# omar-a-aman/Franka-Force-Feedback-MPC

Measured on AMD Instinct MI355X. Metric: FDDP solves/sec, Franka 7-DoF horizon-30 batch=4096, at 1/2/4/8 MI355X, higher is better.
Workload: dtype f64

## Files before the change

franka-force-feedback-mpc_amd/csrc/ffddp_kernels.hip:

```cpp
#include <hip/hip_runtime.h>
#include <sched.h>

#include <cmath>
#include <cstdio>
#include <cstdlib>
#include <cstring>
#include <new>
#include <algorithm>
#include <atomic>
#include <chrono>
#include <condition_variable>
#include <functional>
#include <mutex>
#include <string>
#include <thread>
#include <type_traits>
#include <vector>

#include "ffddp_consts.hpp"
#include "ffddp_group.hpp"
#include "ffddp_plant.hpp"
#include "ffddp_primal_g8.hpp"
#include "ffddp_rollout.hpp"

// ... 28 lines not shown
#define BW_WAVES 1
#endif

struct InstState {
  double preg, cost, dg, dq, stop;
  double ffeas;
  int is_feasible, was_feasible, done, ok, iter, recalc, accepted, bw_ok;
  int n_iters, n_trials, n_retries, n_backward, n_calc, n_forward;
  int n_eval1, n_eval2;
  int n_neg, n_neg_acc;
};

struct Dev {
  int B, N, nx, rec;
  double* rec_buf;
  double* fs;
  double* xs;
  double* us;
  double* K;
  double* k;
  double* w;
  double* xs_try;
  double* us_try;
  double* trial;
  int* trial_fail;
  InstState* st;
  int* alist;
  int* acnt;
  double* trace;
  int trace_it;
};

#define RESERVE_AGPR40() asm volatile("" ::: "a0", "a1", "a2", "a3", "a4", "a5", "a6", "a7", "a8", "a9", "a10", "a11", "a12", "a13", "a14", "a15", "a16", "a17", "a18", "a19", "a20", "a21", "a22", "a23", "a24", "a25", "a26", "a27", "a28", "a29", "a30", "a31", "a32", "a33", "a34", "a35", "a36", "a37", "a38", "a39")

template <class T> using gptr = __attribute__((address_space(1))) T*;

struct ActiveList {
  const int* list;
  int n;
};
__device__ __forceinline__ ActiveList active_list(const Dev& d, int cur) {
  return ActiveList{d.alist + (long)cur * d.B, d.acnt[cur]};
}

constexpr int N_XCD = 8;
__device__ __forceinline__ long xcd_block(long b, long n) {
  if (b >= n) return b;
  const long q = n / N_XCD, r = n % N_XCD;
  const long x = b % N_XCD, i = b / N_XCD;
  return (x < r ? x * (q + 1) : r * (q + 1) + (x - r) * q) + i;
}

__global__ void k_init(const DevConsts* __restrict__ Cg, Dev d, const double* xs_init, const double* us_init,
                       int is_feasible) {
  const DevConsts& C = *Cg;
  const int N = C.N, nx = C.nx;
  const long nX = (long)d.B * (N + 1) * nx;
  const long nU = (long)d.B * N * NU;
  const long nK = (long)d.B * N * NU * nx;
  const long nT = d.trace ? (long)d.B * d.trace_it * FFDDP_TRACE_W : 0;
  for (long i = blockIdx.x * (long)blockDim.x + threadIdx.x; i < nK || i < nT; i += (long)gridDim.x * blockDim.x) {
    if (i < nT) d.trace[i] = __builtin_nan("");
    if (i >= nK) continue;
    if (i < nX) d.xs[i] = xs_init[i];
    if (i < nU) {
      d.us[i] = us_init[i];
      d.k[i] = 0.0;
    }
    d.K[i] = 0.0;
    if (i < d.B) {
      d.alist[i] = (int)i;
      if (i == 0) {
        d.acnt[0] = d.B;
        d.acnt[1] = 0;
        d.acnt[2] = 0;
        d.acnt[3] = 0;
      }
      InstState s;
      s.preg = C.reg_min;
      s.cost = 0.0;
      s.dg = s.dq = 0.0;
      s.stop = __builtin_nan("");
      s.is_feasible = is_feasible;
      s.was_feasible = 0;
      s.done = 0;
      s.ok = 0;
      s.iter = 0;
      s.recalc = 1;
      s.accepted = -1;
      s.bw_ok = 0;
      s.n_iters = s.n_trials = s.n_retries = s.n_backward = s.n_calc = s.n_forward = 0;
      s.n_eval1 = s.n_eval2 = 0;
      s.n_neg = s.n_neg_acc = 0;
      s.ffeas = 0.0;
      d.st[i] = s;
    }
  }
}

struct NodeGroupShared {
  Primal P;
  union {
    double lk[LK_ALLOC];
    double col[14][NDENSE_MAX];
  };
  double colu[7][FFDDP_MAX_NC];
};
struct NodeShared {
  NodeGroupShared g[NODE_GPB];
};

template <int NC, bool FF>
__device__ __forceinline__ void primal_group(const DevConsts& C, const Dev& d, const double* __restrict__ x0,
                                             const double* __restrict__ node_ref, const double* __restrict__ inst_ref,
                                             const uint8_t* __restrict__ surface, int b, int t, Primal* P,
                                             double* lk, const double* __restrict__ xsrc,
                                             const double* __restrict__ usrc) {
  const int N = C.N;
  constexpr int nx = FF ? 21 : 14;
// ... 47 lines not shown
        }
      }
    }
    c += g8_sum(part);
  }
  if (li == 0) {
    rec[rec_off_cost(nx)] = c;
#pragma unroll
    for (int r = 0; r < 3; ++r) rec[rec_off_lam(nx) + r] = (mode == MODE_TERMINAL_X) ? 0.0 : lam[r];
  }
  const bool feas = d.st[b].is_feasible != 0;
  if (J) {
    if (!terminal) {
      double* f = d.fs + ((long)b * (N + 1) + t + 1) * nx;
      const double* yn = xsrc + (long)(t + 1) * nx;
      const double dt = C.dt;
      const double a = P->a[li];
      const double qn = (mode == MODE_TERMINAL_X) ? q : q + (v * dt + a * dt * dt);
      const double vn = (mode == MODE_TERMINAL_X) ? v : v + a * dt;
      f[li] = feas ? 0.0 : qn - yn[li];
      f[7 + li] = feas ? 0.0 : vn - yn[7 + li];
      if (FF) f[14 + li] = feas ? 0.0 : (C.alpha * y[14 + li] + C.beta * usrc[(long)t * NU + li]) - yn[14 + li];
    }
    if (t == 0) {
      double* f = d.fs + (long)b * (N + 1) * nx;
#pragma unroll
      for (int k = 0; k < (FF ? 3 : 2); ++k) f[7 * k + li] = feas ? 0.0 : x0[(long)b * nx + 7 * k + li] - y[7 * k + li];
    }
  }
  if (!FF && commit) {
    double* xr = d.xs + ((long)b * (N + 1) + t) * nx;
    xr[li] = q;
    xr[7 + li] = v;
    if (!terminal) d.us[((long)b * N + t) * NU + li] = cu;
  }
}

template <int NC>
__device__ __forceinline__ double fquad(const double* a, const double* Dd, const double* Do, const double* b) {
  double acc = 0.0;
#pragma unroll
  for (int r = 0; r < NC; ++r) acc += a[r] * Dd[r] * b[r];
  if (NC == 3)
    acc += Do[0] * (a[1] * b[0] + a[0] * b[1]) + Do[1] * (a[2] * b[0] + a[0] * b[2]) +
           Do[2] * (a[2] * b[1] + a[1] * b[2]);
  return acc;
}

template <int NC, bool FF>
__global__ __launch_bounds__(NODE_BLOCK) __attribute__((amdgpu_waves_per_eu(NODE_WAVES))) void k_node(const DevConsts* __restrict__ Cg, Dev d,
                                                      const double* __restrict__ x0,
                                                      const double* __restrict__ node_ref,
                                                      const double* __restrict__ inst_ref,
                                                      const uint8_t* __restrict__ surface, int force_all, int cur) {
  const DevConsts& C = *Cg;
  const int N = C.N;
  constexpr int nx = FF ? 21 : 14;
  constexpr int nc = NC;
  __shared__ NodeShared S;
  const int grp = threadIdx.x / NODE_GROUP, lane = threadIdx.x % NODE_GROUP;
  const int n_work = force_all ? d.B : d.acnt[cur];
  const long blk = xcd_block(blockIdx.x, ((long)n_work * (N + 1) + NODE_GPB - 1) / NODE_GPB);
  const long gnode = blk * NODE_GPB + grp;
  const int slot = (int)(gnode / (N + 1)), t = (int)(gnode % (N + 1));
  int b = slot;
  bool active = slot < d.B;
  if (active && !force_all) {
    const ActiveList al = active_list(d, cur);
    active = slot < al.n;
    b = active ? al.list[slot] : 0;
    if (active) active = (d.st[b].done == 0) && (d.st[b].recalc != 0);
  }
  const long node = (long)b * (N + 1) + t;
  const bool surf = active ? surface[b] != 0 : false;
  const bool terminal = t == N;
  constexpr bool ff = FF;
  const int mode = !terminal ? MODE_RUNNING : (ff ? MODE_TERMINAL_U : MODE_TERMINAL_X);
  const long perX = (long)(N + 1) * nx, perU = (long)N * NU;
  const int acc = active ? d.st[b].accepted : -1;
  const double* xsrc = acc >= 0 ? d.xs_try + ((long)b * NTRIALS + acc) * perX : d.xs + (long)b * perX;
  const double* usrc = acc >= 0 ? d.us_try + ((long)b * NTRIALS + acc) * perU : d.us + (long)b * perU;
  const double* y = xsrc + (long)t * nx;
  const double* ref = node_ref + ((long)b * (N + 1) + t) * 6;
  NodeGroupShared& G = S.g[grp];
  Primal& P = G.P;
  if (active && lane < G8) primal_group<NC, FF>(C, d, x0, node_ref, inst_ref, surface, b, t, &P, G.lk, xsrc, usrc);
  __syncthreads();
  const bool need_u = mode != MODE_TERMINAL_X;
  if (active && lane < 7 && need_u) {
    double dau[NQ], dlamu[3];
    node_tangent_control<NC>(C, surf, P, lane, dau, dlamu);
    double* rec = d.rec_buf + ((long)b * (N + 1) + t) * d.rec;
    for (int i = 0; i < NQ; ++i) rec[rec_off_A() + (14 + lane) * NQ + i] = dau[i];
    for (int r = 0; r < nc; ++r) G.colu[lane][r] = (surf ? dlamu[r] : 0.0);
  }
  double da[NQ], dlam[3], col[NDENSE_MAX], r1[NQ], dh[3];
  if (active && lane < 14) node_tangent_state_links<NC>(C, mode, surf, G.lk, P, lane, r1, dh, col);
  __syncthreads();
  if (active && lane < 14) {
    for (int r = 0; r < 12; ++r) G.col[lane][r] = col[r];
    node_tangent_state_contact<NC>(mode, surf, P, r1, dh, da, dlam, col);
    for (int r = 12; r < 12 + nc; ++r) G.col[lane][r] = col[r];
  }
  __syncthreads();
  if (active) {
    double* rec = d.rec_buf + ((long)b * (N + 1) + t) * d.rec;
    const int nd = 12 + nc;
    const bool scale = mode != MODE_TERMINAL_X;
    const double sc = scale ? C.dt : 1.0;
    const double* D = P.D;
    const double* g = P.g;
    double wy = 0.0, wy2j = 0.0, wy2u = 0.0;
    if (ff) {
      wy = C.w_y;
      wy2j = C.Wy2[lane < 14 ? lane : 0];
      wy2u = C.Wy2[14 + (lane < 7 ? lane : 0)];
      asm volatile("" : "+s"(wy), "+v"(wy2j), "+v"(wy2u));
    }
    if (lane < 14) {
      const int j = lane;
      if (need_u)
        for (int i = 0; i < NQ; ++i) rec[rec_off_A() + j * NQ + i] = da[i];
      double* Lxx = rec + rec_off_Lxx(nx);
      for (int i = 0; i < 14; ++i) {
        double acc = 0.0;
        for (int r = 0; r < 12; ++r) acc += G.col[i][r] * D[r] * col[r];
        acc += fquad<NC>(&G.col[i][12], D + 12, P.Dfo, col + 12);
        if (i == j) acc += P.Dx[j];
        acc *= sc;
        if (ff && i == j) acc += wy * wy2j;
        Lxx[i * nx + j] = acc;
      }
      double lx = 0.0;
      for (int r = 0; r < nd; ++r) lx += col[r] * g[r];
// ... 1473 lines not shown
  if (steplength > C.th_stepdec) s.preg = fmax(s.preg / C.reg_dec, C.reg_min);
  if (steplength <= C.th_stepinc) {
    s.preg = fmin(s.preg * C.reg_inc, C.reg_max);
    if (s.preg == C.reg_max) {
      s.done = 1;
      s.ok = 0;
    }
  }
  if (d.trace && iter < d.trace_it && !s.done) {
    double* r = d.trace + ((long)b * d.trace_it + iter) * FFDDP_TRACE_W;
    r[0] = (double)iter;
    r[1] = s.cost;
    r[2] = s.stop;
    r[3] = -td1;
    r[4] = s.preg;
    r[5] = s.preg;
    r[6] = steplength;
    r[7] = s.ffeas;
    r[8] = tdV;
    r[9] = tdVexp;
  }
  if (!s.done && s.was_feasible && s.stop < C.th_stop) {
    s.done = 1;
    s.ok = 1;
  }
  d.st[b] = s;
  return acc;
}

__global__ __launch_bounds__(64) void k_accept(const DevConsts* __restrict__ Cg, Dev d, int iter, int n1, int cur,
                                               int wide_max) {
  const DevConsts& C = *Cg;
  const ActiveList al = active_list(d, cur);
  const int n1h = n1;
  n1 = first_width(n1, d, cur, wide_max);
  if ((int)blockIdx.x * 64 >= al.n) return;
  const int slot = (int)blockIdx.x * 64 + (int)threadIdx.x;
  const bool has = slot < al.n;
  const int b = has ? al.list[slot] : 0;
  bool cont = false;
  int acc = -1;
  if (has) {
    acc = accept_instance(C, d, b, iter, n1);
    cont = d.st[b].done == 0;
  }
  if (cont && (acc < 0 || acc >= n1h)) d.acnt[2 + (cur ^ 1)] = 1;
  const unsigned long long m = __ballot(cont);
  int base = 0;
  if (threadIdx.x == 0 && m != 0ull) base = atomicAdd(d.acnt + (cur ^ 1), __popcll(m));
  base = __builtin_amdgcn_readfirstlane(base);
  if (cont) d.alist[(long)(cur ^ 1) * d.B + base + __popcll(m & ((1ull << threadIdx.x) - 1ull))] = b;
}

constexpr int COMMIT_IPB = 4;
__global__ __launch_bounds__(64) void k_commit(const DevConsts* __restrict__ Cg, Dev d) {
  const DevConsts& C = *Cg;
  const int q = threadIdx.x / 16, l = threadIdx.x % 16;
  const int b = (int)blockIdx.x * COMMIT_IPB + q;
  if (b >= d.B) return;
  const int acc = d.st[b].accepted;
  if (acc < 0) return;
  const int N = C.N, nx = C.nx;
  const long perX = (long)(N + 1) * nx, perU = (long)N * NU;
  const double* sx = d.xs_try + ((long)b * NTRIALS + acc) * perX;
  const double* su = d.us_try + ((long)b * NTRIALS + acc) * perU;
  double* dx = d.xs + (long)b * perX;
  double* du = d.us + (long)b * perU;
  constexpr int CH = 16;
  for (long base = l; base < perX + perU; base += 16 * CH) {
    double v[CH];
#pragma unroll
    for (int u = 0; u < CH; ++u) {
      const long i = base + 16 * u;
      v[u] = i < perX ? sx[i] : (i < perX + perU ? su[i - perX] : 0.0);
    }
#pragma unroll
    for (int u = 0; u < CH; ++u) {
      const long i = base + 16 * u;
      if (i < perX)
        dx[i] = v[u];
      else if (i < perX + perU)
        du[i - perX] = v[u];
    }
  }
}

template <int NC, bool FF>
__global__ __launch_bounds__(64) void k_finalize(const DevConsts* __restrict__ Cg, Dev d, int maxiter, const double* __restrict__ x0,
                           const double* __restrict__ node_ref, const double* __restrict__ inst_ref,
                           const uint8_t* __restrict__ surface, double* cost, int32_t* iters, uint8_t* ok,
                           double* fn_pred, int32_t* stats) {
  const DevConsts& C = *Cg;
  const int N = C.N;
  constexpr int nx = FF ? 21 : 14;
  const long gid = blockIdx.x * (long)blockDim.x + threadIdx.x;
  const int b = (int)(gid / 2), knot = (int)(gid % 2);
  if (b >= d.B) return;
  const InstState s = d.st[b];
  if (knot == 0) {
    cost[b] = s.cost;
    iters[b] = s.done ? s.iter : maxiter;
    ok[b] = (s.done && s.ok) ? 1 : 0;
    if (stats) {
      stats[(long)b * FFDDP_NSTATS + 0] = s.n_iters;
      stats[(long)b * FFDDP_NSTATS + 1] = s.n_trials;
      stats[(long)b * FFDDP_NSTATS + 2] = s.n_retries;
      stats[(long)b * FFDDP_NSTATS + 3] = s.n_backward;
      stats[(long)b * FFDDP_NSTATS + 4] = s.n_calc;
      stats[(long)b * FFDDP_NSTATS + 5] = s.n_forward;
      stats[(long)b * FFDDP_NSTATS + 6] = s.n_eval1;
      stats[(long)b * FFDDP_NSTATS + 7] = s.n_eval2;
      stats[(long)b * FFDDP_NSTATS + 8] = s.n_neg;
      stats[(long)b * FFDDP_NSTATS + 9] = s.n_neg_acc;
    }
  }
  if (fn_pred == nullptr) return;
  const int t = knot < N ? knot : N - 1;
  if (!surface[b]) {
    fn_pred[(long)b * 2 + knot] = __builtin_nan("");
    return;
  }
  const double* y = d.xs + ((long)b * (N + 1) + t) * nx;
  const double* u = d.us + ((long)b * N + t) * NU;
  const double* ref = node_ref + ((long)b * (N + 1) + t) * 6;
  const double* xreg = inst_ref + (long)b * 21;
  Primal P;
  double yn[21], c;
  node_calc<NC, FF>(C, false, true, y, u, ref, xreg, xreg + 14, x0 + (long)b * nx, P, yn, c);
  fn_pred[(long)b * 2 + knot] = (NC == 1) ? P.lam[0] : P.lam[2];
}

__global__ __launch_bounds__(64) void k_plant(const ffddp_robot* __restrict__ rb, const ffddp_plant_params* __restrict__ pp,
                                              int B, double* __restrict__ q, double* __restrict__ v,
                                              const double* __restrict__ tau, const double* __restrict__ plane,
                                              int integrate, double* __restrict__ obs, int32_t* __restrict__ fail) {
  const int b = blockIdx.x * blockDim.x + threadIdx.x;
  if (b >= B) return;
  double qb[NQ], vb[NQ], tb[NQ], ob[PO_WORDS];
  for (int i = 0; i < NQ; ++i) {
    qb[i] = q[(long)b * NQ + i];
    vb[i] = v[(long)b * NQ + i];
    tb[i] = tau[(long)b * NQ + i];
  }
  const double* pl = plane + (long)b * 6;
  const bool ok = plant_step(*rb, *pp, qb, vb, tb, pl, pl + 3, integrate, ob);
  for (int i = 0; i < NQ; ++i) {
    q[(long)b * NQ + i] = qb[i];
    v[(long)b * NQ + i] = vb[i];
  }
  for (int e = 0; e < PO_WORDS; ++e) obs[(long)b * PO_WORDS + e] = ob[e];
  if (fail) fail[b] = ok ? 0 : 1;
}

__global__ __launch_bounds__(64) void k_gravity(const ffddp_robot* __restrict__ rb, int B, const double* __restrict__ q,
                          double* __restrict__ tau) {
  const int b = blockIdx.x * blockDim.x + threadIdx.x;
  if (b >= B) return;
  gravity_torque(*rb, q + (long)b * NQ, tau + (long)b * NQ);
}

struct TaskTraj {
  double center[3], radius, omega, z_contact, t_approach, t_pre, t_hold;
  double p_start[3], p_pre[3], p_cs[3];
};

__device__ __forceinline__ double smoothstep01(double s) {
  s = fmin(fmax(s, 0.0), 1.0);
  return s * s * (3.0 - 2.0 * s);
}

__device__ __forceinline__ double dsmoothstep01(double s) {
  s = fmin(fmax(s, 0.0), 1.0);
  return 6.0 * s * (1.0 - s);
}

__device__ bool task_base(const TaskTraj& T, double t, double p[3], double v[3]) {
// ... 222 lines not shown
    uint64_t seen = 0;
    for (;;) {
      {
        std::unique_lock<std::mutex> lk(mu_);
        cv_.wait(lk, [&] { return stop_ || (gen_ != seen && work_ != nullptr); });
        if (stop_) return;
        seen = gen_;
      }
      drain();
    }
  }
  std::vector<std::thread> th_;
  std::mutex mu_;
  std::condition_variable cv_, done_cv_;
  const std::vector<CopyJob>* work_ = nullptr;
  std::atomic<size_t> next_{0};
  size_t left_ = 0;
  uint64_t gen_ = 0;
  bool stop_ = false;
};

struct ffddp_handle {
  int device = 0;
  int max_batch = 0;
  DevConsts hc{};
  DevConsts* dc = nullptr;
  ffddp_robot* drb = nullptr;
  Dev d{};
  double *in_x0 = nullptr, *in_nref = nullptr, *in_iref = nullptr, *in_xs = nullptr, *in_us = nullptr;
  uint8_t* in_surf = nullptr;
  double *out_xs = nullptr, *out_us = nullptr, *out_K = nullptr, *out_cost = nullptr, *out_fn = nullptr;
  int32_t *out_iters = nullptr, *out_stats = nullptr;
  uint8_t* out_ok = nullptr;
  std::string err;
  char* stage = nullptr;
  size_t stage_bytes = 0;
  std::vector<hipEvent_t> hdone;
  CopyPool* pool = nullptr;
  double* trace = nullptr;
  int trace_it = 0;
  std::vector<ffddp_plan*> plans;
  hipEvent_t last_done = nullptr;
  bool last_done_set = false;
  int nstreams = 4;
  std::vector<hipStream_t> streams;
  std::vector<hipEvent_t> sev;
  std::vector<hipEvent_t> stg;
  bool caller_slice = true;
  int stagger = -1;
  int fw_first = 4;
  std::vector<int> fw_sched{2, 2, 2, 2};
  int bw_late_max = -1;
  int bw_w2_max = -1;
  int n_simd = 1024;
  bool fw_fill = true;
  int fw_long = 0;
  int fw_wide_max = -1;
  int ls_row_max = -1;
  bool prof = false;
  int prof_mask = 0;
  std::vector<hipEvent_t> ev_pool;
  size_t ev_used = 0;
  std::vector<int> ev_class;
  double prof_ms[FFDDP_NKERNELS] = {0};
  int64_t prof_n[FFDDP_NKERNELS] = {0};
};

namespace {

bool stream_pool_acquire(int device, int n, std::vector<hipStream_t>& out);
void stream_pool_release(int device, int n);


int fail(ffddp_handle* h, int code, const std::string& msg) {
  if (h) h->err = msg;
  return code;
}

#define HIPCHK(h, expr)                                                                    \
  do {                                                                                     \
    hipError_t e_ = (expr);                                                                \
    if (e_ != hipSuccess)                                                                  \
      return fail(h, FFDDP_E_DEVICE, std::string(#expr) + ": " + hipGetErrorString(e_));  \
  } while (0)

template <class T> int dalloc(ffddp_handle* h, T** p, size_t n) {
  if (hipMalloc((void**)p, n * sizeof(T) + 64) != hipSuccess) {
    *p = nullptr;
    return fail(h, FFDDP_E_OOM, "hipMalloc failed");
  }
  return 0;
}

void free_all(ffddp_handle* h) {
  void* ps[] = {h->dc, h->drb, h->d.alist, h->d.acnt, h->d.rec_buf, h->d.fs, h->d.xs, h->d.us, h->d.K, h->d.k, h->d.w, h->d.xs_try,
                h->d.us_try, h->d.trial, h->d.trial_fail, h->d.st, h->in_x0, h->in_nref, h->in_iref, h->in_xs,
                h->in_us, h->in_surf, h->out_xs, h->out_us, h->out_K, h->out_cost, h->out_fn, h->out_iters,
                h->out_stats, h->out_ok};
  for (void* p : ps)
    if (p) (void)hipFree(p);
  if (h->trace) (void)hipFree(h->trace);
  if (h->stage) (void)hipHostFree(h->stage);
}

struct ProfScope {
  ffddp_handle* h;
// ... 40 lines not shown
  d.acnt += 4 * k;
  if (d.trace) d.trace += (long)b0 * d0.trace_it * FFDDP_TRACE_W;
  return d;
}

template <int NC, bool FF>
int launch_solve_t(ffddp_handle* h, int B, const double* x0, const double* nref, const double* iref,
                 const uint8_t* surf, const double* xs_init, const double* us_init, int maxiter, int is_feasible,
                 double* xs, double* us, double* K, double* cost, int32_t* iters, uint8_t* ok, double* fn_pred,
                 int32_t* stats, hipStream_t s, HostIO* io) {
  const int N = h->hc.N, nx = h->hc.nx;
  int S = h->nstreams;
  if (B < 64 * S) S = 1;
  if (S > 1) {
    if ((int)h->streams.size() < S && !stream_pool_acquire(h->device, S, h->streams))
      return fail(h, FFDDP_E_DEVICE, "hipStreamCreate failed");
    while ((int)h->sev.size() < S + 1) {
      hipEvent_t e;
      HIPCHK(h, hipEventCreateWithFlags(&e, hipEventDisableTiming));
      h->sev.push_back(e);
    }
    while ((int)h->stg.size() < S) {
      hipEvent_t e;
      HIPCHK(h, hipEventCreateWithFlags(&e, hipEventDisableTiming));
      h->stg.push_back(e);
    }
  }
  const int Bs = (B + S - 1) / S;
  const int stagger = S == 1 ? 0 : (h->stagger >= 0 ? h->stagger : (Bs > h->n_simd / S ? 1 : 0));
  struct Slice {
    Dev d;
    hipStream_t s;
    int b0, B;
  };
  Slice sl[8];
  Dev dbase = h->d;
  if (!io) {
    dbase.xs = xs;
    dbase.us = us;
    dbase.K = K;
  }
  for (int k = 0; k < S; ++k) {
    sl[k].b0 = k * Bs;
    sl[k].B = (B - sl[k].b0) < Bs ? (B - sl[k].b0) : Bs;
    sl[k].d = dev_slice(dbase, sl[k].b0, sl[k].B, k);
    sl[k].s = (S > 1 && !(h->caller_slice && k == S - 1)) ? h->streams[k] : s;
  }
  if (S > 1) {
    HIPCHK(h, hipEventRecord(h->sev[0], s));
    for (int k = 0; k < S; ++k)
      if (sl[k].s != s) HIPCHK(h, hipStreamWaitEvent(sl[k].s, h->sev[0], 0));
  }
  const long nxl = nx, N1 = N + 1;
  if (io) {
    io->ns = S;
    for (int k = 0; k < S; ++k) {
      io->b0[k] = sl[k].b0;
      io->bk[k] = sl[k].B;
    }
  }
  auto enqueue_in = [&](int k) -> int {
    for (int i = 0; i < io->n_in; ++i) {
      const size_t o = (size_t)sl[k].b0 * io->in[i].per_inst;
      HIPCHK(h, hipMemcpyAsync((char*)io->in[i].dev + o, (const char*)io->in[i].host + o,
                               (size_t)sl[k].B * io->in[i].per_inst, hipMemcpyHostToDevice, sl[k].s));
    }
    return 0;
  };
  auto enqueue_init = [&](int k) {
    ProfScope p(h, sl[k].s, KC_INIT);
    const long b0 = sl[k].b0;
    hipLaunchKernelGGL(k_init, dim3(1024), dim3(256), 0, sl[k].s, h->dc, sl[k].d, xs_init + b0 * N1 * nxl,
                       us_init + b0 * (long)N * NU, is_feasible);
  };
  auto enqueue_iter = [&](int k, int it) -> int {
    const Dev& d = sl[k].d;
    const hipStream_t ss = sl[k].s;
    const int Bk = sl[k].B;
    const long b0 = sl[k].b0;
    const double* x0k = x0 + b0 * nxl;
    const double* nrefk = nref + b0 * N1 * 6;
    const double* irefk = iref + b0 * 21;
    const uint8_t* surfk = surf + b0;
    const long nodes = (long)Bk * (N + 1);
    if (it == 0 && k > 0 && stagger) HIPCHK(h, hipStreamWaitEvent(ss, h->stg[k - 1], 0));
    if (it == 0 && stagger == 2 && k + 1 < S) HIPCHK(h, hipEventRecord(h->stg[k], ss));
    {
      ProfScope p(h, ss, KC_NODE);
      hipLaunchKernelGGL((k_node<NC, FF>), dim3((int)((nodes + NODE_GPB - 1) / NODE_GPB)), dim3(NODE_BLOCK), 0, ss,
                         h->dc, d, x0k, nrefk, irefk, surfk, 0, it & 1);
    }
    if (it == 0 && stagger == 1 && k + 1 < S) HIPCHK(h, hipEventRecord(h->stg[k], ss));
    {
      ProfScope p(h, ss, KC_BACKWARD);
      const int lmax = h->bw_late_max >= 0 ? h->bw_late_max : h->n_simd / S;
      const bool small = Bk <= h->n_simd / S;
      const int w2auto = small ? h->n_simd / (2 * S) : (FF ? 0 : lmax);
      const int w2max = std::min(lmax, h->bw_w2_max >= 0 ? h->bw_w2_max : w2auto);
      if (lmax < Bk)
        hipLaunchKernelGGL((k_backward_w<FF>), dim3(Bk), dim3(64), 0, ss, h->dc, d, it, it & 1, lmax, w2max);
      if (lmax > w2max && w2max < Bk)
        hipLaunchKernelGGL((k_backward_w<FF, true>), dim3(lmax < Bk ? lmax : Bk), dim3(64), 0, ss, h->dc, d, it, it & 1,
                           lmax, w2max);
      if (w2max > 0) {
        const dim3 g2(w2max < Bk ? w2max : Bk);
        if constexpr (!FF) {
          if (!small) {
            hipLaunchKernelGGL((k_backward_w2<FF, 2>), g2, dim3(128), 0, ss, h->dc, d, it, it & 1, w2max);
          } else {
            hipLaunchKernelGGL((k_backward_w2<FF, 1>), g2, dim3(128), 0, ss, h->dc, d, it, it & 1, w2max);
          }
        } else {
          hipLaunchKernelGGL((k_backward_w2<FF, 1>), g2, dim3(128), 0, ss, h->dc, d, it, it & 1, w2max);
        }
      }
    }
    int n1 = NTRIALS;
    {
      n1 = it < (int)h->fw_sched.size() ? h->fw_sched[it] : h->fw_first;
      if (h->fw_fill) n1 = std::max(n1, std::min(NTRIALS, 8 * h->n_simd / std::max(B, 1)));
      if (h->fw_fill && h->fw_long > 0 && N >= h->fw_long && n1 >= 8) n1 = NTRIALS;
      const int wide = h->fw_wide_max >= 0 ? h->fw_wide_max : h->n_simd / S;
      const long g1 = std::max((long)Bk * n1, (long)std::min(Bk, wide) * NTRIALS);
      const int row_max = (h->ls_row_max >= 0 ? h->ls_row_max : 4 * h->n_simd / S) *
                          (h->ls_row_max < 0 && Bk > h->n_simd / S ? 0 : 1);
      const bool row_only = row_max > 0 && (long)Bk * NTRIALS <= (long)row_max;
      auto fw = [&](int tr0, int ntr, int more) {
        const long groups = more ? (long)Bk * ntr : g1;
        if (!row_only) {
          const dim3 grid((unsigned)((groups * G8 + 63) / 64));
          hipLaunchKernelGGL((k_forward_g8<NC, FF, false>), grid, dim3(64), 0, ss, h->dc, d, x0k, nrefk, irefk,
                             surfk, tr0, ntr, more, it & 1, wide, row_max);
        }
        if (row_max > 0) {
          const long rg = std::min(groups, (long)row_max);
          const dim3 grid((unsigned)((rg * 16 + 63) / 64));
          hipLaunchKernelGGL((k_forward_g8<NC, FF, true>), grid, dim3(64), 0, ss, h->dc, d, x0k, nrefk, irefk,
                             surfk, tr0, ntr, more, it & 1, wide, row_max);
        }
      };
      {
        ProfScope p(h, ss, KC_FORWARD);
        fw(0, n1, 0);
      }
      if (n1 < NTRIALS) {
        ProfScope p(h, ss, KC_FORWARD2);
        fw(n1, NTRIALS - n1, 1);
      }
    }
    {
      ProfScope p(h, ss, KC_ACCEPT);
      hipLaunchKernelGGL(k_accept, dim3((Bk + 63) / 64), dim3(64), 0, ss, h->dc, d, it, n1, it & 1,
                         h->fw_wide_max >= 0 ? h->fw_wide_max : h->n_simd / S);
    }
    return 0;
  };
  const size_t bxs = (size_t)(N + 1) * nx * sizeof(double);
  const size_t bus = (size_t)N * NU * sizeof(double);
  const size_t bks = (size_t)N * NU * nx * sizeof(double);
  auto enqueue_tail = [&](int k) -> int {
    const Dev& d = sl[k].d;
    const hipStream_t ss = sl[k].s;
    const long b0 = sl[k].b0;
    const int Bk = sl[k].B;
    {
      ProfScope p(h, ss, KC_COMMIT);
      hipLaunchKernelGGL(k_commit, dim3((Bk + COMMIT_IPB - 1) / COMMIT_IPB), dim3(64), 0, ss, h->dc, d);
    }
    {
      ProfScope p(h, ss, KC_FINALIZE);
      hipLaunchKernelGGL((k_finalize<NC, FF>), dim3((2 * Bk + 63) / 64), dim3(64), 0, ss, h->dc, d, maxiter,
                         x0 + b0 * nxl, nref + b0 * N1 * 6, iref + b0 * 21, surf + b0, cost + b0, iters + b0, ok + b0,
                         fn_pred ? fn_pred + 2 * b0 : nullptr, stats ? stats + b0 * FFDDP_NSTATS : nullptr);
    }
    if (io) {
      io->ss[k] = ss;
      io->dxs[k] = d.xs;
      io->dus[k] = d.us;
      io->dK[k] = d.K;
      if (!io->defer_out) {
        HIPCHK(h, hipMemcpyAsync(xs + b0 * N1 * nxl, d.xs, bxs * Bk, hipMemcpyDefault, ss));
        HIPCHK(h, hipMemcpyAsync(us + b0 * (long)N * NU, d.us, bus * Bk, hipMemcpyDefault, ss));
        HIPCHK(h, hipMemcpyAsync(K + b0 * (long)N * NU * nx, d.K, bks * Bk, hipMemcpyDefault, ss));
      }
      for (int i = 0; i < io->n_out; ++i) {
        const size_t o = (size_t)b0 * io->out[i].per_inst;
        HIPCHK(h, hipMemcpyAsync((char*)io->out[i].host + o, (const char*)io->out[i].dev + o,
                                 (size_t)Bk * io->out[i].per_inst, hipMemcpyDeviceToHost, ss));
      }
      if (!io->defer_out) HIPCHK(h, hipEventRecord(io->done[k], ss));
    }
    return 0;
  };
  if (io && io->stage) {
    for (int k = 0; k < S; ++k) {
      if (const int rc = io->stage(k)) return rc;
      if (const int rc = enqueue_in(k)) return rc;
      enqueue_init(k);
      for (int it = 0; it < maxiter; ++it)
        if (const int rc = enqueue_iter(k, it)) return rc;
      if (const int rc = enqueue_tail(k)) return rc;
    }
  } else {
    if (io)
      for (int k = 0; k < S; ++k)
        if (const int rc = enqueue_in(k)) return rc;
    for (int k = 0; k < S; ++k) enqueue_init(k);
    for (int it = 0; it < maxiter; ++it)
      for (int k = 0; k < S; ++k)
        if (const int rc = enqueue_iter(k, it)) return rc;
    for (int k = 0; k < S; ++k)
      if (const int rc = enqueue_tail(k)) return rc;
  }
  if (hipGetLastError() != hipSuccess) return fail(h, FFDDP_E_DEVICE, "kernel launch failed");
  if (S > 1) {
    for (int k = 0; k < S; ++k) {
      if (sl[k].s == s) continue;
      HIPCHK(h, hipEventRecord(h->sev[1 + k], sl[k].s));
      HIPCHK(h, hipStreamWaitEvent(s, h->sev[1 + k], 0));
    }
  }
  return 0;
}

int launch_solve(ffddp_handle* h, int B, const double* x0, const double* nref, const double* iref,
                 const uint8_t* surf, const double* xs_init, const double* us_init, int maxiter, int is_feasible,
                 double* xs, double* us, double* K, double* cost, int32_t* iters, uint8_t* ok, double* fn_pred,
                 int32_t* stats, hipStream_t s, HostIO* io = nullptr) {
  const bool ff = h->hc.variant == FFDDP_FORCE_FEEDBACK;
  const int nc = h->hc.nc;
#define FFDDP_LS(NC_, FF_) \
  launch_solve_t<NC_, FF_>(h, B, x0, nref, iref, surf, xs_init, us_init, maxiter, is_feasible, xs, us, K, cost, iters, ok, fn_pred, stats, s, io)
  if (nc == 1) return ff ? FFDDP_LS(1, true) : FFDDP_LS(1, false);
  return ff ? FFDDP_LS(3, true) : FFDDP_LS(3, false);
#undef FFDDP_LS
}

template <int NC, bool FF>
void launch_node(ffddp_handle* h, Dev d, int B, hipStream_t s, int force_all) {
  const long nodes = (long)B * (h->hc.N + 1);
  hipLaunchKernelGGL((k_node<NC, FF>), dim3((int)((nodes + NODE_GPB - 1) / NODE_GPB)), dim3(NODE_BLOCK), 0, s, h->dc,
                     d, h->in_x0, h->in_nref, h->in_iref, h->in_surf, force_all, 0);
}

struct StreamPool {
  std::vector<hipStream_t> s;
  int refs = 0;
};
std::mutex g_pool_mu;
StreamPool g_pool[64];

bool stream_pool_acquire(int device, int n, std::vector<hipStream_t>& out) {
  std::lock_guard<std::mutex> lk(g_pool_mu);
  StreamPool& p = g_pool[device & 63];
  while ((int)p.s.size() < n) {
    hipStream_t st;
    if (hipStreamCreateWithFlags(&st, hipStreamNonBlocking) != hipSuccess) return false;
    p.s.push_back(st);
  }
  const int had = (int)out.size();
  out.assign(p.s.begin(), p.s.begin() + n);
  p.refs += n - had;
  return true;
}

void stream_pool_release(int device, int n) {
  std::lock_guard<std::mutex> lk(g_pool_mu);
  StreamPool& p = g_pool[device & 63];
  p.refs -= n;
  if (p.refs <= 0) {
    for (hipStream_t st : p.s) (void)hipStreamDestroy(st);
    p.s.clear();
    p.refs = 0;
  }
}

bool host_pinned(const void* p) {
  hipPointerAttribute_t a;
  if (hipPointerGetAttributes(&a, p) != hipSuccess) {
    (void)hipGetLastError();
    return false;
  }
  return a.type == hipMemoryTypeHost;
}

int copy_threads() {
  if (const char* e = std::getenv("FFDDP_COPY_THREADS")) {
    const int v = std::atoi(e);
    return v < 1 ? 1 : (v > 64 ? 64 : v);
  }
  cpu_set_t cs;
  int n = 8;
  if (sched_getaffinity(0, sizeof(cs), &cs) == 0) n = CPU_COUNT(&cs);
  return n < 1 ? 1 : (n > 16 ? 16 : n);
}

bool valid_cfg(const ffddp_ocp_config& c) {
  return (c.variant == FFDDP_CLASSICAL || c.variant == FFDDP_FORCE_FEEDBACK) && c.horizon >= 1 &&
         c.horizon <= 4096 && (c.nc == 1 || c.nc == 3) && c.dt > 0.0;
}

}

extern "C" {

int ffddp_create(const ffddp_robot* robot, const ffddp_ocp_config* cfg, int device, int max_batch,
                 ffddp_handle** out) {
  if (!robot || !cfg || !out || max_batch < 1) return FFDDP_E_INVALID;
  *out = nullptr;
  if (!valid_cfg(*cfg)) return FFDDP_E_INVALID;
  ffddp_handle* h = new (std::nothrow) ffddp_handle();
  if (!h) return FFDDP_E_OOM;
  h->device = device;
  h->max_batch = max_batch;
  fill_consts(*robot, *cfg, h->hc);
  if (hipSetDevice(device) != hipSuccess) {
    delete h;
    return FFDDP_E_DEVICE;
  }
  const long B = max_batch, N = cfg->horizon, nx = h->hc.nx;
  Dev& d = h->d;
  d.N = (int)N;
  d.nx = (int)nx;
  d.rec = rec_size((int)nx);
  if (d.rec != rec_words((int)nx)) {
    delete h;
    return FFDDP_E_INVALID;
  }
  {
    int cu = 0;
    if (hipDeviceGetAttribute(&cu, hipDeviceAttributeMultiprocessorCount, device) == hipSuccess && cu > 0)
      h->n_simd = 4 * cu;
    const char* ns = std::getenv("FFDDP_STREAMS");
    if (ns) {
      const int v = std::atoi(ns);
      h->nstreams = v < 1 ? 1 : (v > 8 ? 8 : v);
    }
    if (const char* bl = std::getenv("FFDDP_BW_LATE_MAX")) h->bw_late_max = std::atoi(bl);
    if (const char* bw2 = std::getenv("FFDDP_BW_W2_MAX")) h->bw_w2_max = std::atoi(bw2);
    if (const char* ff = std::getenv("FFDDP_FW_FILL")) h->fw_fill = std::atoi(ff) != 0;
    if (const char* fl = std::getenv("FFDDP_FW_LONG")) h->fw_long = std::atoi(fl);
    if (const char* fwm = std::getenv("FFDDP_FW_WIDE_MAX")) h->fw_wide_max = std::atoi(fwm);
    if (const char* lrm = std::getenv("FFDDP_LS_ROW_MAX")) h->ls_row_max = std::atoi(lrm);
    if (const char* fsch = std::getenv("FFDDP_FW_SCHED")) {
      h->fw_sched.clear();
      for (const char* p = fsch; *p;) {
        const int v = std::atoi(p);
        h->fw_sched.push_back(v < 1 ? 1 : (v > NTRIALS ? NTRIALS : v));
        while (*p && *p != ',') ++p;
        if (*p == ',') ++p;
      }
    }
    if (const char* sg = std::getenv("FFDDP_STAGGER")) h->stagger = std::atoi(sg);
    if (const char* cs = std::getenv("FFDDP_CALLER_SLICE")) h->caller_slice = std::atoi(cs) != 0;
    const char* f1 = std::getenv("FFDDP_FW_FIRST");
    if (f1) {
      const int v = std::atoi(f1);
      h->fw_first = v < 1 ? 1 : (v > NTRIALS ? NTRIALS : v);
    }
  }
  if (h->nstreams > 1 && !stream_pool_acquire(h->device, h->nstreams, h->streams)) {
    delete h;
    return FFDDP_E_DEVICE;
  }
  int rc = 0;
  rc |= dalloc(h, &h->dc, 1);
  rc |= dalloc(h, &h->drb, 1);
  rc |= dalloc(h, &d.rec_buf, (size_t)B * (N + 1) * d.rec);
  rc |= dalloc(h, &d.fs, (size_t)B * (N + 1) * nx);
  rc |= dalloc(h, &d.xs, (size_t)B * (N + 1) * nx);
  rc |= dalloc(h, &d.us, (size_t)B * N * NU);
  rc |= dalloc(h, &d.K, (size_t)B * N * NU * nx);
  rc |= dalloc(h, &d.k, (size_t)B * N * NU);
  rc |= dalloc(h, &d.w, (size_t)B * (N + 1) * nx);
  rc |= dalloc(h, &d.xs_try, (size_t)B * NTRIALS * (N + 1) * nx);
  rc |= dalloc(h, &d.us_try, (size_t)B * NTRIALS * N * NU);
  rc |= dalloc(h, &d.trial, (size_t)B * NTRIALS * 2);
  rc |= dalloc(h, &d.trial_fail, (size_t)B * NTRIALS);
  rc |= dalloc(h, &d.st, (size_t)B);
  rc |= dalloc(h, &d.alist, (size_t)B * 2);
  rc |= dalloc(h, &d.acnt, (size_t)4 * 8);
  rc |= dalloc(h, &h->in_x0, (size_t)B * nx);
  rc |= dalloc(h, &h->in_nref, (size_t)B * (N + 1) * 6);
  rc |= dalloc(h, &h->in_iref, (size_t)B * 21);
  rc |= dalloc(h, &h->in_xs, (size_t)B * (N + 1) * nx);
  rc |= dalloc(h, &h->in_us, (size_t)B * N * NU);
  rc |= dalloc(h, &h->in_surf, (size_t)B);
  rc |= dalloc(h, &h->out_xs, (size_t)B * (N + 1) * nx);
  rc |= dalloc(h, &h->out_us, (size_t)B * N * NU);
  rc |= dalloc(h, &h->out_K, (size_t)B * N * NU * nx);
  rc |= dalloc(h, &h->out_cost, (size_t)B);
  rc |= dalloc(h, &h->out_fn, (size_t)B * 2);
// ... 510 lines not shown
  HIPCHK(h, hipSetDevice(h->device));
  HIPCHK(h, hipDeviceSynchronize());
  HIPCHK(h, hipMemcpy(h->dc, &c, sizeof(DevConsts), hipMemcpyHostToDevice));
  h->hc = c;
  return 0;
}

int ffddp_trace_enable(ffddp_handle* h, int max_iters) {
  if (!h || max_iters < 0) return FFDDP_E_INVALID;
  if (!h->plans.empty())
    return fail(h, FFDDP_E_INVALID, "solve plans of this handle are alive: destroy them before ffddp_trace_enable");
  HIPCHK(h, hipSetDevice(h->device));
  if (h->trace) {
    HIPCHK(h, hipDeviceSynchronize());
    (void)hipFree(h->trace);
  }
  h->trace = nullptr;
  h->trace_it = 0;
  h->d.trace = nullptr;
  h->d.trace_it = 0;
  if (max_iters == 0) return 0;
  if (int rc = dalloc(h, &h->trace, (size_t)h->max_batch * max_iters * FFDDP_TRACE_W)) return rc;
  h->trace_it = max_iters;
  h->d.trace = h->trace;
  h->d.trace_it = max_iters;
  return 0;
}

int ffddp_trace_read(ffddp_handle* h, int B, double* out) {
  if (!h || !out || B < 0 || B > h->max_batch) return FFDDP_E_INVALID;
  if (!h->trace) return fail(h, FFDDP_E_INVALID, "trace not enabled (ffddp_trace_enable)");
  HIPCHK(h, hipSetDevice(h->device));
  HIPCHK(h, hipDeviceSynchronize());
  HIPCHK(h, hipMemcpy(out, h->trace, (size_t)B * h->trace_it * FFDDP_TRACE_W * 8, hipMemcpyDeviceToHost));
  return 0;
}

int ffddp_calc_diff(ffddp_handle* h, int B, const double* x0, const double* node_ref, const double* inst_ref,
                    const uint8_t* surface, const double* xs, const double* us, double* Fx, double* Fu, double* Lx,
                    double* Lu, double* Lxx, double* Lxu, double* Luu, double* cost, double* xnext, double* lam) {
  if (!h) return FFDDP_E_INVALID;
  if (B < 1 || B > h->max_batch) return fail(h, FFDDP_E_CAPACITY, "bad B");
  HIPCHK(h, hipSetDevice(h->device));
  const int N = h->hc.N, nx = h->hc.nx, R = h->d.rec;
  const bool ff = h->hc.variant == FFDDP_FORCE_FEEDBACK;
  Dev d = h->d;
  d.B = B;
  HIPCHK(h, hipMemcpy(h->in_x0, x0, (size_t)B * nx * 8, hipMemcpyHostToDevice));
  HIPCHK(h, hipMemcpy(h->in_nref, node_ref, (size_t)B * (N + 1) * 6 * 8, hipMemcpyHostToDevice));
  HIPCHK(h, hipMemcpy(h->in_iref, inst_ref, (size_t)B * 21 * 8, hipMemcpyHostToDevice));
  HIPCHK(h, hipMemcpy(h->in_surf, surface, (size_t)B, hipMemcpyHostToDevice));
  HIPCHK(h, hipMemcpy(h->in_xs, xs, (size_t)B * (N + 1) * nx * 8, hipMemcpyHostToDevice));
  HIPCHK(h, hipMemcpy(h->in_us, us, (size_t)B * N * NU * 8, hipMemcpyHostToDevice));
  hipLaunchKernelGGL(k_init, dim3(1024), dim3(256), 0, nullptr, h->dc, d, h->in_xs, h->in_us, 0);
  if (h->hc.nc == 1)
    ff ? launch_node<1, true>(h, d, B, nullptr, 1) : launch_node<1, false>(h, d, B, nullptr, 1);
  else
    ff ? launch_node<3, true>(h, d, B, nullptr, 1) : launch_node<3, false>(h, d, B, nullptr, 1);
  HIPCHK(h, hipGetLastError());
  HIPCHK(h, hipDeviceSynchronize());
  std::vector<double> rec((size_t)B * (N + 1) * R), fsv((size_t)B * (N + 1) * nx);
  HIPCHK(h, hipMemcpy(rec.data(), d.rec_buf, rec.size() * 8, hipMemcpyDeviceToHost));
  HIPCHK(h, hipMemcpy(fsv.data(), d.fs, fsv.size() * 8, hipMemcpyDeviceToHost));
  const double dt = h->hc.dt;
  for (int b = 0; b < B; ++b) {
    for (int t = 0; t <= N; ++t) {
      const double* r = rec.data() + ((size_t)b * (N + 1) + t) * R;
      const size_t nt = (size_t)b * (N + 1) + t;
      for (int i = 0; i < nx; ++i) Lx[nt * nx + i] = r[rec_off_Lx(nx) + i];
      for (int e = 0; e < nx * nx; ++e) Lxx[nt * nx * nx + e] = r[rec_off_Lxx(nx) + e];
      cost[nt] = r[rec_off_cost(nx)];
      for (int c = 0; c < 3; ++c) lam[nt * 3 + c] = r[rec_off_lam(nx) + c];
      if (t == N) continue;
      const size_t rt = (size_t)b * N + t;
      const double* A = r + rec_off_A();
      for (int i = 0; i < NU; ++i) Lu[rt * NU + i] = r[rec_off_Lu(nx) + i];
      for (int e = 0; e < nx * NU; ++e) Lxu[rt * nx * NU + e] = r[rec_off_Lxu(nx) + e];
      for (int e = 0; e < NU * NU; ++e) Luu[rt * NU * NU + e] = r[rec_off_Luu(nx) + e];
      for (int i = 0; i < nx; ++i) {
        for (int j = 0; j < nx; ++j) {
          double v = (i == j) ? 1.0 : 0.0;
          if (i < 14 && j < (ff ? 21 : 14)) {
            v += (i < 7 ? dt * dt : dt) * A[j * NQ + (i % 7)];
            if (i < 7 && j == i + 7) v += dt;
          }
          if (ff && i >= 14) v = (i == j) ? h->hc.alpha : 0.0;
          Fx[rt * nx * nx + i * nx + j] = v;
        }
        for (int kk = 0; kk < NU; ++kk) {
          double v;
          if (!ff)
            v = (i < 7 ? dt * dt : dt) * A[(14 + kk) * NQ + (i % 7)];
          else
            v = (i >= 14 && i - 14 == kk) ? h->hc.beta : 0.0;
          Fu[rt * nx * NU + i * NU + kk] = v;
        }
      }
      for (int i = 0; i < nx; ++i)
        xnext[rt * nx + i] = xs[((size_t)b * (N + 1) + t + 1) * nx + i] + fsv[((size_t)b * (N + 1) + t + 1) * nx + i];
    }
  }
  return 0;
}

int ffddp_frame_placement(const ffddp_robot* robot, const double* q, double* R, double* p) {
  if (!robot || !q || !R || !p) return FFDDP_E_INVALID;
  RBOut<double> o;
  const double zero[NQ] = {0, 0, 0, 0, 0, 0, 0};
  rb_pass<double, false, false>(*robot, q, zero, zero, nullptr, o, nullptr);
  for (int i = 0; i < 9; ++i) R[i] = o.Ree.m[i];
  p[0] = o.pee.x;
// ... 172 lines not shown
```

Measured before the change: 563,500.

## Skip initial trajectory copy and fuse commit into finalize kernel

```diff
diff --git a/franka-force-feedback-mpc_amd/csrc/ffddp_kernels.hip b/franka-force-feedback-mpc_amd/csrc/ffddp_kernels.hip
--- a/franka-force-feedback-mpc_amd/csrc/ffddp_kernels.hip
+++ b/franka-force-feedback-mpc_amd/csrc/ffddp_kernels.hip
@@ -104,7 +104,7 @@
 }
 
 __global__ void k_init(const DevConsts* __restrict__ Cg, Dev d, const double* xs_init, const double* us_init,
-                       int is_feasible) {
+                       int is_feasible, int copy) {
   const DevConsts& C = *Cg;
   const int N = C.N, nx = C.nx;
   const long nX = (long)d.B * (N + 1) * nx;
@@ -114,9 +114,9 @@
   for (long i = blockIdx.x * (long)blockDim.x + threadIdx.x; i < nK || i < nT; i += (long)gridDim.x * blockDim.x) {
     if (i < nT) d.trace[i] = __builtin_nan("");
     if (i >= nK) continue;
-    if (i < nX) d.xs[i] = xs_init[i];
+    if (copy && i < nX) d.xs[i] = xs_init[i];
     if (i < nU) {
-      d.us[i] = us_init[i];
+      if (copy) d.us[i] = us_init[i];
       d.k[i] = 0.0;
     }
     d.K[i] = 0.0;
@@ -270,7 +270,9 @@
                                                       const double* __restrict__ x0,
                                                       const double* __restrict__ node_ref,
                                                       const double* __restrict__ inst_ref,
-                                                      const uint8_t* __restrict__ surface, int force_all, int cur) {
+                                                      const uint8_t* __restrict__ surface, int force_all, int cur,
+                                                      const double* __restrict__ xs0,
+                                                      const double* __restrict__ us0) {
   const DevConsts& C = *Cg;
   const int N = C.N;
   constexpr int nx = FF ? 21 : 14;
@@ -296,8 +298,8 @@
   const int mode = !terminal ? MODE_RUNNING : (ff ? MODE_TERMINAL_U : MODE_TERMINAL_X);
   const long perX = (long)(N + 1) * nx, perU = (long)N * NU;
   const int acc = active ? d.st[b].accepted : -1;
-  const double* xsrc = acc >= 0 ? d.xs_try + ((long)b * NTRIALS + acc) * perX : d.xs + (long)b * perX;
-  const double* usrc = acc >= 0 ? d.us_try + ((long)b * NTRIALS + acc) * perU : d.us + (long)b * perU;
+  const double* xsrc = acc >= 0 ? d.xs_try + ((long)b * NTRIALS + acc) * perX : (xs0 ? xs0 : d.xs) + (long)b * perX;
+  const double* usrc = acc >= 0 ? d.us_try + ((long)b * NTRIALS + acc) * perU : (us0 ? us0 : d.us) + (long)b * perU;
   const double* y = xsrc + (long)t * nx;
   const double* ref = node_ref + ((long)b * (N + 1) + t) * 6;
   NodeGroupShared& G = S.g[grp];
@@ -1877,39 +1879,8 @@
   if (cont) d.alist[(long)(cur ^ 1) * d.B + base + __popcll(m & ((1ull << threadIdx.x) - 1ull))] = b;
 }
 
-constexpr int COMMIT_IPB = 4;
-__global__ __launch_bounds__(64) void k_commit(const DevConsts* __restrict__ Cg, Dev d) {
-  const DevConsts& C = *Cg;
-  const int q = threadIdx.x / 16, l = threadIdx.x % 16;
-  const int b = (int)blockIdx.x * COMMIT_IPB + q;
-  if (b >= d.B) return;
-  const int acc = d.st[b].accepted;
-  if (acc < 0) return;
-  const int N = C.N, nx = C.nx;
-  const long perX = (long)(N + 1) * nx, perU = (long)N * NU;
-  const double* sx = d.xs_try + ((long)b * NTRIALS + acc) * perX;
-  const double* su = d.us_try + ((long)b * NTRIALS + acc) * perU;
-  double* dx = d.xs + (long)b * perX;
-  double* du = d.us + (long)b * perU;
-  constexpr int CH = 16;
-  for (long base = l; base < perX + perU; base += 16 * CH) {
-    double v[CH];
-#pragma unroll
-    for (int u = 0; u < CH; ++u) {
-      const long i = base + 16 * u;
-      v[u] = i < perX ? sx[i] : (i < perX + perU ? su[i - perX] : 0.0);
-    }
-#pragma unroll
-    for (int u = 0; u < CH; ++u) {
-      const long i = base + 16 * u;
-      if (i < perX)
-        dx[i] = v[u];
-      else if (i < perX + perU)
-        du[i - perX] = v[u];
-    }
-  }
-}
-
+constexpr int FIN_LANES = 16;
+constexpr int FIN_IPB = 64 / FIN_LANES;
 template <int NC, bool FF>
 __global__ __launch_bounds__(64) void k_finalize(const DevConsts* __restrict__ Cg, Dev d, int maxiter, const double* __restrict__ x0,
                            const double* __restrict__ node_ref, const double* __restrict__ inst_ref,
@@ -1918,10 +1889,37 @@
   const DevConsts& C = *Cg;
   const int N = C.N;
   constexpr int nx = FF ? 21 : 14;
-  const long gid = blockIdx.x * (long)blockDim.x + threadIdx.x;
-  const int b = (int)(gid / 2), knot = (int)(gid % 2);
+  const int l = threadIdx.x % FIN_LANES;
+  const int b = (int)blockIdx.x * FIN_IPB + (int)threadIdx.x / FIN_LANES;
   if (b >= d.B) return;
   const InstState s = d.st[b];
+  const int acc = s.accepted;
+  const long perX = (long)(N + 1) * nx, perU = (long)N * NU;
+  const double* sx = acc >= 0 ? d.xs_try + ((long)b * NTRIALS + acc) * perX : d.xs + (long)b * perX;
+  const double* su = acc >= 0 ? d.us_try + ((long)b * NTRIALS + acc) * perU : d.us + (long)b * perU;
+  if (acc >= 0) {
+    double* dx = d.xs + (long)b * perX;
+    double* du = d.us + (long)b * perU;
+    constexpr int CH = 16;
+    for (long base = l; base < perX + perU; base += FIN_LANES * CH) {
+      double v[CH];
+#pragma unroll
+      for (int u = 0; u < CH; ++u) {
+        const long i = base + FIN_LANES * u;
+        v[u] = i < perX ? sx[i] : (i < perX + perU ? su[i - perX] : 0.0);
+      }
+#pragma unroll
+      for (int u = 0; u < CH; ++u) {
+        const long i = base + FIN_LANES * u;
+        if (i < perX)
+          dx[i] = v[u];
+        else if (i < perX + perU)
+          du[i - perX] = v[u];
+      }
+    }
+  }
+  const int knot = l;
+  if (knot >= 2) return;
   if (knot == 0) {
     cost[b] = s.cost;
     iters[b] = s.done ? s.iter : maxiter;
@@ -1945,8 +1943,8 @@
     fn_pred[(long)b * 2 + knot] = __builtin_nan("");
     return;
   }
-  const double* y = d.xs + ((long)b * (N + 1) + t) * nx;
-  const double* u = d.us + ((long)b * N + t) * NU;
+  const double* y = sx + (long)t * nx;
+  const double* u = su + (long)t * NU;
   const double* ref = node_ref + ((long)b * (N + 1) + t) * 6;
   const double* xreg = inst_ref + (long)b * 21;
   Primal P;
@@ -2275,6 +2273,7 @@
   std::vector<int> fw_sched{2, 2, 2, 2};
   int bw_late_max = -1;
   int bw_w2_max = -1;
+  int bw_tail_waves = 2;
   int n_simd = 1024;
   bool fw_fill = true;
   int fw_long = 0;
@@ -2421,6 +2420,9 @@
       if (sl[k].s != s) HIPCHK(h, hipStreamWaitEvent(sl[k].s, h->sev[0], 0));
   }
   const long nxl = nx, N1 = N + 1;
+  const bool inplace_x = xs_init == dbase.xs, inplace_u = us_init == dbase.us;
+  const bool guess_direct = maxiter > 0 && !inplace_x && !inplace_u;
+  const int init_copy = !guess_direct && !(inplace_x && inplace_u);
   if (io) {
     io->ns = S;
     for (int k = 0; k < S; ++k) {
@@ -2440,7 +2442,7 @@
     ProfScope p(h, sl[k].s, KC_INIT);
     const long b0 = sl[k].b0;
     hipLaunchKernelGGL(k_init, dim3(1024), dim3(256), 0, sl[k].s, h->dc, sl[k].d, xs_init + b0 * N1 * nxl,
-                       us_init + b0 * (long)N * NU, is_feasible);
+                       us_init + b0 * (long)N * NU, is_feasible, init_copy);
   };
   auto enqueue_iter = [&](int k, int it) -> int {
     const Dev& d = sl[k].d;
@@ -2457,7 +2459,9 @@
     {
       ProfScope p(h, ss, KC_NODE);
       hipLaunchKernelGGL((k_node<NC, FF>), dim3((int)((nodes + NODE_GPB - 1) / NODE_GPB)), dim3(NODE_BLOCK), 0, ss,
-                         h->dc, d, x0k, nrefk, irefk, surfk, 0, it & 1);
+                         h->dc, d, x0k, nrefk, irefk, surfk, 0, it & 1,
+                         it == 0 && guess_direct ? xs_init + b0 * N1 * nxl : nullptr,
+                         it == 0 && guess_direct ? us_init + b0 * (long)N * NU : nullptr);
     }
     if (it == 0 && stagger == 1 && k + 1 < S) HIPCHK(h, hipEventRecord(h->stg[k], ss));
     {
@@ -2474,7 +2478,7 @@
       if (w2max > 0) {
         const dim3 g2(w2max < Bk ? w2max : Bk);
         if constexpr (!FF) {
-          if (!small) {
+          if (!small && h->bw_tail_waves == 2) {
             hipLaunchKernelGGL((k_backward_w2<FF, 2>), g2, dim3(128), 0, ss, h->dc, d, it, it & 1, w2max);
           } else {
             hipLaunchKernelGGL((k_backward_w2<FF, 1>), g2, dim3(128), 0, ss, h->dc, d, it, it & 1, w2max);
@@ -2533,12 +2537,8 @@
     const long b0 = sl[k].b0;
     const int Bk = sl[k].B;
     {
-      ProfScope p(h, ss, KC_COMMIT);
-      hipLaunchKernelGGL(k_commit, dim3((Bk + COMMIT_IPB - 1) / COMMIT_IPB), dim3(64), 0, ss, h->dc, d);
-    }
-    {
       ProfScope p(h, ss, KC_FINALIZE);
-      hipLaunchKernelGGL((k_finalize<NC, FF>), dim3((2 * Bk + 63) / 64), dim3(64), 0, ss, h->dc, d, maxiter,
+      hipLaunchKernelGGL((k_finalize<NC, FF>), dim3((Bk + FIN_IPB - 1) / FIN_IPB), dim3(64), 0, ss, h->dc, d, maxiter,
                          x0 + b0 * nxl, nref + b0 * N1 * 6, iref + b0 * 21, surf + b0, cost + b0, iters + b0, ok + b0,
                          fn_pred ? fn_pred + 2 * b0 : nullptr, stats ? stats + b0 * FFDDP_NSTATS : nullptr);
     }
@@ -2606,10 +2606,10 @@
 }
 
 template <int NC, bool FF>
-void launch_node(ffddp_handle* h, Dev d, int B, hipStream_t s, int force_all) {
+void launch_node(ffddp_handle* h, Dev d, int B, hipStream_t s, int force_all, const double* xs0, const double* us0) {
   const long nodes = (long)B * (h->hc.N + 1);
   hipLaunchKernelGGL((k_node<NC, FF>), dim3((int)((nodes + NODE_GPB - 1) / NODE_GPB)), dim3(NODE_BLOCK), 0, s, h->dc,
-                     d, h->in_x0, h->in_nref, h->in_iref, h->in_surf, force_all, 0);
+                     d, h->in_x0, h->in_nref, h->in_iref, h->in_surf, force_all, 0, xs0, us0);
 }
 
 struct StreamPool {
@@ -2707,6 +2707,7 @@
     }
     if (const char* bl = std::getenv("FFDDP_BW_LATE_MAX")) h->bw_late_max = std::atoi(bl);
     if (const char* bw2 = std::getenv("FFDDP_BW_W2_MAX")) h->bw_w2_max = std::atoi(bw2);
+    if (const char* btw = std::getenv("FFDDP_BW_TAIL_WAVES")) h->bw_tail_waves = std::atoi(btw) == 1 ? 1 : 2;
     if (const char* ff = std::getenv("FFDDP_FW_FILL")) h->fw_fill = std::atoi(ff) != 0;
     if (const char* fl = std::getenv("FFDDP_FW_LONG")) h->fw_long = std::atoi(fl);
     if (const char* fwm = std::getenv("FFDDP_FW_WIDE_MAX")) h->fw_wide_max = std::atoi(fwm);
@@ -3323,11 +3324,11 @@
   HIPCHK(h, hipMemcpy(h->in_surf, surface, (size_t)B, hipMemcpyHostToDevice));
   HIPCHK(h, hipMemcpy(h->in_xs, xs, (size_t)B * (N + 1) * nx * 8, hipMemcpyHostToDevice));
   HIPCHK(h, hipMemcpy(h->in_us, us, (size_t)B * N * NU * 8, hipMemcpyHostToDevice));
-  hipLaunchKernelGGL(k_init, dim3(1024), dim3(256), 0, nullptr, h->dc, d, h->in_xs, h->in_us, 0);
+  hipLaunchKernelGGL(k_init, dim3(1024), dim3(256), 0, nullptr, h->dc, d, h->in_xs, h->in_us, 0, 0);
   if (h->hc.nc == 1)
-    ff ? launch_node<1, true>(h, d, B, nullptr, 1) : launch_node<1, false>(h, d, B, nullptr, 1);
+    ff ? launch_node<1, true>(h, d, B, nullptr, 1, h->in_xs, h->in_us) : launch_node<1, false>(h, d, B, nullptr, 1, h->in_xs, h->in_us);
   else
-    ff ? launch_node<3, true>(h, d, B, nullptr, 1) : launch_node<3, false>(h, d, B, nullptr, 1);
+    ff ? launch_node<3, true>(h, d, B, nullptr, 1, h->in_xs, h->in_us) : launch_node<3, false>(h, d, B, nullptr, 1, h->in_xs, h->in_us);
   HIPCHK(h, hipGetLastError());
   HIPCHK(h, hipDeviceSynchronize());
   std::vector<double> rec((size_t)B * (N + 1) * R), fsv((size_t)B * (N + 1) * nx);
```

New measurement: 567,200, median of 6. Within noise of the previous version (+0.7%).
